# Griffan/FASTQuick

Measured on AMD Instinct MI355X. Metric: paired_150bp_reads_aligned_per_sec, higher is better.
Workload: dtype u32

## Files before the change

fastquick_amd/csrc/fq_align.cpp:

```cpp
#include <algorithm>
#include <atomic>
#include <ctime>
#include <chrono>
#include <climits>
#include <cstdint>
#include <cmath>
#include <cstdio>
#include <cstdlib>
#include <cstring>
#include <memory>
#include <string>
#include <unordered_map>
#include <mutex>
#include <thread>
#include <vector>
#include <pthread.h>
#include <sched.h>

#include "../../include/fastquick_amd.h"
#include "fq_backend.h"
#include "fq_index.h"
#include "fq_pipeline.h"
#include "fq_pool.h"
#include "fq_text_batch.h"
// ... 385 lines not shown
  else if (k == "device_turns") c->kn.device_turns = (int)v;
  else if (k == "device_turn_min") c->kn.device_turn_min = v;
  else if (k == "device_turn_slots") c->kn.device_turn_slots = (int)std::max<int64_t>(1, v);
  else if (k == "gap_round2_waves") c->kn.gap_round2_waves = (int)v;
  else if (k == "gap_round2_lane_major") c->kn.gap_round2_lane_major = (int)v;
  else if (k == "gap_round1_refill") c->kn.gap_round1_refill = (int)v;
  else if (k == "gap_round2_refill") c->kn.gap_round2_refill = (int)v;
  else if (k == "sw_wave_max") c->kn.sw_wave_max = (int)v;
  else if (k == "host_threads") c->kn.host_threads = (int)v;
  else if (k == "host_par_min") c->kn.host_par_min = (size_t)v;
  else if (k == "packed_bulk_min") c->kn.packed_bulk_min = v;
  else if (k == "md_mask_min") c->kn.md_mask_min = v;
  else if (k == "trace") c->kn.trace = (int)v;
  else if (k == "gap_order_asc") t->gap_order_asc = (int)v;
  else if (k == "gap_waves_per_cu") t->gap_waves_per_cu = (int)v;
  else if (k == "gap_coop_waves") t->gap_coop_waves = (int)v;
  else if (k == "gap_refill_min") t->gap_refill_min = (int)v;
  else if (k == "filter_no_turns") t->filter_no_turns = (int)v;
  else if (k == "prep_priority") t->prep_priority = (int)v;
  else if (k == "refine_lanes") t->refine_lanes = (int)v;
  else if (k == "gap_generic_opts") t->gap_generic_opts = (int)v;
  else if (k == "sw_serial_reverse") t->sw_serial_reverse = (int)v;
  else if (k == "width_both_strands") t->width_both_strands = (int)v;
  else if (k == "spin_sync") t->spin_sync = (int)v;
  else return FQ_EINVAL;
  return FQ_OK;
}

extern "C" void fq_stats_get(const fq_ctx_t *c, fq_stats_t *out) { if (c && out) *out = c->stats; }
extern "C" void fq_stats_reset(fq_ctx_t *c) { if (c) memset(&c->stats, 0, sizeof c->stats); }

#define CK(expr)                                                  \
  do {                                                            \
    if ((expr)) { c->err = std::string(#expr) + ": " + fqdev::last_error(); return FQ_ENODEV; } \
  } while (0)
#define CKM(expr)                                                 \
  do {                                                            \
    if (!(expr)) { c->err = std::string("out of device memory: ") + #expr; return FQ_ENOMEM; } \
  } while (0)

static int h2d_staged(fq_ctx *c, void *dst, const void *src, size_t bytes) {
  if (!bytes) return 0;
  void *p = c->arena.alloc(bytes);
  if (!p) { c->err = "out of pinned host memory"; return FQ_ENOMEM; }
  memcpy(p, src, bytes);
  if (fqdev::copy_pinned(dst, p, bytes, 1)) { c->err = std::string("h2d: ") + fqdev::last_error(); return FQ_ENODEV; }
// ... 712 lines not shown
    FqGapArgs gb = gap_args(c, b2, g, T2, (int32_t)cnt);
    gb.aln += (size_t)n2_total * T2.aln_cap; gb.n_aln += n2_total; gb.status += n2_total;
    gb.refill_min = 16;
    CK(fqdev::launch_gap(gb));
    CK(fqdev::stream_aux(0));
    n2_total += cnt;
  }
  CK(fqdev::stream_join());
  fqdev::time_end(FQ_K_GAP);
  *n2 = n2_total;
  return FQ_OK;
}

int stageA_search(Call &K) {
  fq_ctx *c = K.c;
  const fq_opts_t &o = c->o;
  SearchBufs &b = c->sb[0];
  const int n_search = K.n_search, max_len_all = K.max_len_all;
  c->st.aln.p = c->p_aln.p; c->st.aln.n = 0;
  par_assign(K.aln_off, (size_t)n_search + 1, (uint64_t)0, K.host_threads, K.par_min);
  par_assign(K.aln_n, (size_t)n_search, (uint32_t)0, K.host_threads, K.par_min);
  CKM(c->d_aoff.ensure((size_t)n_search + 1) && c->d_an.ensure((size_t)n_search + 1) && c->d_hits.ensure(1));
  CK(fqdev::dzero(c->d_an.p, ((size_t)n_search + 1) * 4));
  const SearchGeom g = {(max_len_all + 1 + 7) & ~7, (max_len_all + 1 + FQ_POS_PAD + 7) & ~7,
                        (c->maxdiff_lut[max_len_all] + 1) * o.s_mm + o.max_gapo * o.s_gapo + o.max_gape * o.s_gape + 1};
  const uint32_t exact_pool = (uint32_t)std::min<uint64_t>(4ull * (uint64_t)o.max_entries + 4096ull, 0x7fffffffull);
  const FqGapTier lane_tier = {c->kn.gap_pool, 32u, 0, 0, c->kn.gap_long_pops, c->kn.gap_long_always, 0, 0};
  const FqGapTier wave_tier = {262144u, 512u, 0, 1, 0u, 0, 0, 0}, exact_tier = {exact_pool, 8192u, 1, 1, 0u, 0, 0, 0};
  vector<FqGapTier> tiers;
  vector<size_t> chunk_reads;
  if (c->kn.gap_nogap_min >= 0 && !c->kn.gap_long_always && !(o.mode & FQ_MODE_NONSTOP) && c->kn.gap_pool <= 65535u) {
    FqGapTier t = lane_tier; t.nogap = 1; t.long_pops = 0; tiers.push_back(t); chunk_reads.push_back((size_t)8 << 20);
  }
  const size_t n_first_tiers = tiers.size();
  tiers.push_back(lane_tier); chunk_reads.push_back((size_t)8 << 20);
  tiers.push_back(wave_tier); chunk_reads.push_back((size_t)1 << 20);
  tiers.push_back(exact_tier); chunk_reads.push_back(4096);
  vector<int32_t> &work = c->cv.work, &next_work = c->cv.next_work;
  work.resize((size_t)n_search);
  parallel_chunks((size_t)n_search, K.host_threads, K.par_min, [&](size_t lo, size_t hi, int) { for (size_t s = lo; s < hi; ++s) work[s] = (int32_t)s; });
  bool ran_nogap = false;
  size_t n_hard = 0;
  vector<uint8_t> bound_of;
  for (size_t tier = 0; tier < tiers.size() && !work.empty(); ++tier) {
    FqGapTier T = tiers[tier];
    if (T.nogap && (int64_t)work.size() < c->kn.gap_nogap_min) continue;
    if (T.nogap) ran_nogap = true;
// ... 1367 lines not shown
```

fastquick_amd/csrc/fq_backend.h:

```cpp
#pragma once
#include "fq_kernels.h"
#include "fq_records.h"
#include "fq_frontend.h"
#include "fq_emit.h"
#include "fq_deflate.h"
#include "fq_sort.h"
#include "fq_bamin.h"

namespace fqdev {

struct State;
struct Tune {
  int gap_coop_waves = 0;
  int gap_waves_per_cu = 0, gap_refill_min = 0, gap_order_asc = 0, filter_no_turns = 0, refine_lanes = 0;
  int spin_sync = 0;
  int gap_generic_opts = 0;
  int width_both_strands = 0;
  int prep_priority = 0;
  int sw_serial_reverse = 0;
};
int runtime_configure(int hw_queues, int blocking_waits);
int device_count();
State *state_create(int device_ordinal);
void state_destroy(State *s);
int bind(State *s);
Tune *tune(State *s);
const char *last_error();
bool is_real_gpu();
void device_turn_begin(int slots = 1);
void device_turn_end();

void *dmalloc(size_t bytes);
void dfree(void *p);
void *hmalloc(size_t bytes);
void hfree(void *p);
int h2d(void *dst, const void *src, size_t bytes);
int d2h(void *dst, const void *src, size_t bytes);
int copy_pinned(void *dst, const void *src, size_t bytes, int to_device);
int d2d(void *dst, const void *src, size_t bytes);
int dzero(void *dst, size_t bytes);
int dfill(void *dst, int byte, size_t bytes);
int sync();
// ... 61 lines not shown
```

fastquick_amd/csrc/fq_device.hip:

```cpp
#include <hip/hip_runtime.h>
#include <hip/hip_ext.h>

#include <algorithm>
#include <condition_variable>
#include <atomic>
#include <cstdio>
#include <cstdlib>
#include <cstring>
#include <mutex>
#include <string>
#include <unordered_map>
#include <vector>
#include <sys/mman.h>
#include <sys/syscall.h>
#include <unistd.h>

#include "fq_backend.h"
#define FQ_PC_KERNELS
#include "fq_popcon.h"
#define FQ_SVD_KERNELS
#include "fq_svd.h"

namespace fqdev {

// ... 129 lines not shown
  }
  for (auto &p : s->pending) { (void)hipEventDestroy(p.a); (void)hipEventDestroy(p.b); }
  for (auto e : s->free_events) (void)hipEventDestroy(e);
  for (auto e : s->copy_done) if (e) (void)hipEventDestroy(e);
  if (s->prep_done) (void)hipEventDestroy(s->prep_done);
  if (s->scan_tmp) (void)hipFree(s->scan_tmp);
  if (s->cmp_cnt) (void)hipFree(s->cmp_cnt);
  if (s->cmp_off) (void)hipFree(s->cmp_off);
  if (s->stream) (void)hipStreamDestroy(s->stream);
  delete s;
}
Tune *tune(State *s) { return &s->tune; }
int bind(State *s) {
  if (!s) { g_err = "no device state"; return -3; }
  if (g_cur != s) { FQ_HIP(hipSetDevice(s->device)); g_cur = s; }
  return 0;
}

void *dmalloc(size_t bytes) {
  void *p = nullptr;
  if (hipMalloc(&p, bytes ? bytes : 16) != hipSuccess) { g_err = "hipMalloc failed (" + std::to_string(bytes) + " B)"; return nullptr; }
  return p;
}
void dfree(void *p) { if (p) (void)hipFree(p); }
static const size_t kRegisterMin = (size_t)4 << 20;
static std::mutex g_reg_mu;
static std::unordered_map<void *, size_t> g_registered;
static int device_numa_node(int dev) {
  static std::mutex mu;
  static std::unordered_map<int, int> cache;
  std::lock_guard<std::mutex> lk(mu);
  auto it = cache.find(dev);
  if (it != cache.end()) return it->second;
  int node = -1;
  char bus[64] = {0};
  if (hipDeviceGetPCIBusId(bus, (int)sizeof bus, dev) == hipSuccess) {
    for (char *c = bus; *c; ++c) if (*c >= 'A' && *c <= 'F') *c = (char)(*c - 'A' + 'a');
    const std::string path = std::string("/sys/bus/pci/devices/") + bus + "/numa_node";
    if (FILE *f = fopen(path.c_str(), "r")) { if (fscanf(f, "%d", &node) != 1) node = -1; fclose(f); }
  } else (void)hipGetLastError();
  cache[dev] = node;
  return node;
}
static void prefer_node(void *m, size_t len, int node) {
  if (node < 0 || node >= 1024) return;
  unsigned long mask[16] = {0};
  mask[node / (8 * sizeof(unsigned long))] |= 1ul << (node % (8 * sizeof(unsigned long)));
// ... 154 lines not shown
    g_cur->free_events.push_back(p.b);
  }
  g_cur->pending.swap(later);
}

static inline unsigned nblk(uint64_t n, unsigned b) { return (unsigned)((n + b - 1) / b); }

__global__ void __launch_bounds__(256) k_prep(FqPrepArgs a) {
  const int r = blockIdx.x * blockDim.x + threadIdx.x;
  if (r < a.n_reads) fq_prep_thread(a, r);
}
extern __shared__ __align__(16) unsigned char fq_dyn_lds[];
__global__ void __launch_bounds__(256) k_width(FqWidthArgs a) {
  uint8_t *seed_bits = (uint8_t *)fq_dyn_lds;
  const int w = blockIdx.x * blockDim.x + threadIdx.x;
  if (w < a.n_work) fq_width_read(a, w, seed_bits + threadIdx.x, 256);
}
__global__ void __launch_bounds__(256) k_width_strand(FqWidthArgs a) {
  uint8_t *seed_bits = (uint8_t *)fq_dyn_lds;
  const int xcd = blockIdx.x & 7, strand = xcd >> 2;
  const int q = (int)(blockIdx.x >> 3) * 4 + (xcd & 3);
  const int w = q * 256 + threadIdx.x;
  if (w < a.n_work) fq_width_strand(a, w, strand, seed_bits + threadIdx.x, 256);
}
struct FqQueueFetch {
  uint32_t *cursor;
  int n_work;
  __device__ uint32_t operator()(uint32_t n) const { return atomicAdd(cursor, n); }
};
#if defined(FQ_GAP_WPE)
#define FQ_GAP_OCC __attribute__((amdgpu_waves_per_eu(FQ_GAP_WPE, FQ_GAP_WPE)))
#else
#define FQ_GAP_OCC
#endif
#if defined(FQ_NOGAP_WPE)
#define FQ_NOGAP_OCC __attribute__((amdgpu_waves_per_eu(FQ_NOGAP_WPE, FQ_NOGAP_WPE)))
#define FQ_NOGAP_WAVES_PER_CU (4 * FQ_NOGAP_WPE)
#else
#define FQ_NOGAP_OCC FQ_GAP_OCC
#define FQ_NOGAP_WAVES_PER_CU 16
#endif
struct FqQueueFetch2 {
  uint32_t *cursor;
  const uint32_t *split;
  uint32_t n_work;
  int pref, seg, n_seg;
// ... 21 lines not shown
}
__global__ void __launch_bounds__(64) FQ_NOGAP_OCC k_gap_nogap_lds(FqGapArgs a) {
  uint16_t *heads = (uint16_t *)fq_dyn_lds;
  FqGapStoreLds st = {heads + threadIdx.x, 64, (uint32_t *)(heads + 64 * a.o.n_buckets) + threadIdx.x};
  fq_gap_lanes<true>(a, st, FQ_LANE_FETCH(a), (int)(blockIdx.x * 64 + threadIdx.x));
}
__global__ void __launch_bounds__(64) FQ_GAP_OCC k_gap_persist_stock(FqGapArgs a) {
  uint16_t *heads = (uint16_t *)fq_dyn_lds;
  FqGapStoreLds st = {heads + threadIdx.x, 64, (uint32_t *)(heads + 64 * a.o.n_buckets) + threadIdx.x};
  fq_gap_lanes<false, FqOptsStock>(a, st, FQ_LANE_FETCH(a), (int)(blockIdx.x * 64 + threadIdx.x));
}
__global__ void __launch_bounds__(64) FQ_NOGAP_OCC k_gap_nogap_stock(FqGapArgs a) {
  uint16_t *heads = (uint16_t *)fq_dyn_lds;
  FqGapStoreLds st = {heads + threadIdx.x, 64, (uint32_t *)(heads + 64 * a.o.n_buckets) + threadIdx.x};
  fq_gap_lanes<true, FqOptsStock>(a, st, FQ_LANE_FETCH(a), (int)(blockIdx.x * 64 + threadIdx.x));
}
__global__ void __launch_bounds__(64) k_gap_persist(FqGapArgs a) {
  FqGapStoreGlobal st = {nullptr, {}};
  fq_gap_lanes<false>(a, st, FQ_LANE_FETCH(a), (int)(blockIdx.x * 64 + threadIdx.x));
}
__global__ void __launch_bounds__(64) k_gap_coop(FqGapArgs a) {
  __shared__ uint32_t heads[2 * FQ_MAX_BUCKETS];
  fq_gap_coop_wave(a, heads, FqQueueFetch{a.queue, a.n_work}, (int)blockIdx.x);
}
__global__ void __launch_bounds__(256) k_sa(FqSaArgs a) {
  const uint64_t q = (uint64_t)blockIdx.x * blockDim.x + threadIdx.x;
  if (q < a.n_rows) fq_sa_thread(a, q);
}
template <bool PACKED>
__device__ __forceinline__ uint8_t fq_trace_get(const uint8_t *trace, int W, int j, int i) {
  if (!PACKED) return trace[(size_t)j * W + i];
  return (uint8_t)((trace[(size_t)j * ((W + 1) >> 1) + (i >> 1)] >> (4 * (i & 1))) & 15);
}
template <bool PACKED>
__device__ int fq_global_align_wave(const uint8_t *s1, int len1, const uint8_t *s2, int len2, int band, int gap_end,
                                    int *RM, int *RI, int *RD, uint8_t *trace, uint8_t *ops, int *n_ops, int *fi, int *fj) {
  const int lane = threadIdx.x;
  if (len1 == 0 || len2 == 0) { *n_ops = 0; return 0; }
  const FqBand g = fq_band(len1, len2, band, gap_end);
  if (lane == 0) {
    FqCell left;
    left.M = 0; left.I = left.D = FQ_NEG_INF;
    RM[0] = 0; RI[0] = RD[0] = FQ_NEG_INF;
    for (int i = 1; i < g.b1; ++i) {
      uint8_t tb;
      left = fq_band_row0(g, left, tb);
// ... 695 lines not shown
  if (t < a.n_rows) fq_trim_thread(a, t);
}
int launch_trim(const FqTrimArgs &a) {
  FQ_PRE();
  if (a.n_rows <= 0) return 0;
  hipLaunchKernelGGL(k_trim, dim3(nblk((uint64_t)a.n_rows, 256)), dim3(256), 0, g_stream, a);
  FQ_HIP(hipGetLastError());
  return 0;
}
__global__ void __launch_bounds__(256) k_trim_all(FqTrimAllArgs a) {
  const int r = blockIdx.x * blockDim.x + threadIdx.x;
  if (r < a.n_reads) fq_trim_all_thread(a, r);
}
int launch_trim_all(const FqTrimAllArgs &a) {
  FQ_PRE();
  if (a.n_reads <= 0) return 0;
  hipLaunchKernelGGL(k_trim_all, dim3(nblk((uint64_t)a.n_reads, 256)), dim3(256), 0, g_stream, a);
  FQ_HIP(hipGetLastError());
  return 0;
}
int launch_width(const FqWidthArgs &a) {
  FQ_PRE();
  if (a.n_work <= 0) return 0;
  hipEvent_t e0, e1;
  kernel_events(FQ_K_WIDTH_KERNEL, &e0, &e1);
  if (!g_cur->tune.width_both_strands) {
    const unsigned per_strand = nblk((uint64_t)a.n_work, 256);
    const unsigned grid = ((per_strand + 3) / 4) * 8;
    hipExtLaunchKernelGGL(k_width_strand, dim3(grid), dim3(256), (size_t)a.o.seed_len * 256, g_stream, e0, e1, 0, a);
  } else
  hipExtLaunchKernelGGL(k_width, dim3(nblk((uint64_t)a.n_work, 256)), dim3(256), (size_t)2 * (size_t)a.o.seed_len * 256, g_stream, e0, e1, 0, a);
  FQ_HIP(hipGetLastError());
  return 0;
}
__global__ void __launch_bounds__(256) k_order_count(const uint8_t *bid_end, int n, int n_hard, uint32_t *cnt) {
  __shared__ uint32_t h[FQ_ORDER_KEYS];
  if (threadIdx.x < FQ_ORDER_KEYS) h[threadIdx.x] = 0;
  __syncthreads();
  const int w = blockIdx.x * blockDim.x + threadIdx.x;
  if (w < n) atomicAdd(&h[fq_order_key(bid_end, w, n_hard)], 1u);
  __syncthreads();
  if (threadIdx.x < FQ_ORDER_KEYS && h[threadIdx.x]) atomicAdd(&cnt[threadIdx.x], h[threadIdx.x]);
}
__global__ void __launch_bounds__(256) k_order_scatter(const uint8_t *bid_end, int n, int n_hard, uint32_t *cnt, int32_t *order, int asc) {
  __shared__ uint32_t h[FQ_ORDER_KEYS], base[FQ_ORDER_KEYS];
  if (threadIdx.x < FQ_ORDER_KEYS) h[threadIdx.x] = 0;
  __syncthreads();
  const int w = blockIdx.x * blockDim.x + threadIdx.x;
  int key = 0;
  uint32_t rank = 0;
  if (w < n) { key = fq_order_key(bid_end, w, n_hard); rank = atomicAdd(&h[key], 1u); }
  __syncthreads();
// ... 72 lines not shown
  hipEvent_t e0, e1;
  kernel_events(a.tier.nogap ? FQ_K_GAP_NOGAP : FQ_K_GAP_KERNEL, &e0, &e1);
  if (a.tier.coop) {
    hipExtLaunchKernelGGL(k_gap_coop, dim3((unsigned)gap_lane_slots(a)), dim3(64), 0, g_stream, e0, e1, 0, a);
  } else {
    const size_t lds = (size_t)64 * (size_t)a.o.n_buckets * 2 + (size_t)64 * FQ_COLD_N * 4;
    const unsigned grid = (unsigned)gap_lane_slots(a) / 64u;
    if (a.tier.exact) { g_err = "launch_gap: the exact tier is the wavefront kernel's"; return -1; }
    const bool stock = FqOptsStock::matches(a.o) && !g_cur->tune.gap_generic_opts;
    if (a.tier.pool_cap <= 65535u && a.tier.nogap) hipExtLaunchKernelGGL(stock ? k_gap_nogap_stock : k_gap_nogap_lds, dim3(grid), dim3(64), lds, g_stream, e0, e1, 0, a);
    else if (a.tier.pool_cap <= 65535u) hipExtLaunchKernelGGL(stock ? k_gap_persist_stock : k_gap_persist_lds, dim3(grid), dim3(64), lds, g_stream, e0, e1, 0, a);
    else hipExtLaunchKernelGGL(k_gap_persist, dim3(grid), dim3(64), 0, g_stream, e0, e1, 0, a);
  }
  FQ_HIP(hipGetLastError());
  return 0;
}
int launch_pack_aln(const FqAln *aln, const uint32_t *n_aln, const uint64_t *off, uint32_t cap, uint32_t n_work, FqAln *packed) {
  FQ_PRE();
  if (!n_work) return 0;
  hipLaunchKernelGGL(k_pack_aln, dim3(nblk(n_work, 256)), dim3(256), 0, g_stream, aln, n_aln, off, cap, n_work, packed);
  FQ_HIP(hipGetLastError());
  return 0;
}
int launch_sa(const FqSaArgs &a) {
  FQ_PRE();
  if (!a.n_rows) return 0;
  hipEvent_t e0, e1;
  kernel_events(FQ_K_SA_KERNEL, &e0, &e1);
  hipExtLaunchKernelGGL(k_sa, dim3(nblk(a.n_rows, 256)), dim3(256), 0, g_stream, e0, e1, 0, a);
  FQ_HIP(hipGetLastError());
  return 0;
}
static const size_t kLdsBudget = 150 * 1024;
int launch_sw(const FqSwArgs &a) {
  FQ_PRE();
  if (a.n_task <= 0) return 0;
  const FqSwLds L(a.RL, a.QL);
  if (L.bytes(false) > kLdsBudget) { g_err = "SW window too large for LDS (" + std::to_string(a.RL) + " bases)"; return -5; }
  FqSwArgs b = a;
  b.trace_in_lds = (L.bytes(true) <= kLdsBudget && a.n_task <= 256) ? 1 : 0;
  b.serial_reverse = g_cur->tune.sw_serial_reverse;
  hipEvent_t e0, e1;
  kernel_events(FQ_K_SW_KERNEL, &e0, &e1);
  hipExtLaunchKernelGGL(k_sw_wave, dim3((unsigned)a.n_task), dim3(64), L.bytes(b.trace_in_lds), g_stream, e0, e1, 0, b);
  FQ_HIP(hipGetLastError());
  ++dp_launches[b.trace_in_lds ? FQ_DP_SW_WAVE_LDS : FQ_DP_SW_WAVE_GLOBAL];
  return 0;
}
__global__ void __launch_bounds__(64) k_sw_thread(FqSwArgs a) {
// ... 50 lines not shown
FQ_REC_KERNEL(k_pair_scatter, fq_pair_scatter_thread)
FQ_REC_KERNEL(k_xa_count, fq_xa_count_thread)
FQ_REC_KERNEL(k_xa_fill, fq_xa_fill_thread)
FQ_REC_KERNEL(k_sw_plan, fq_sw_plan_thread)
FQ_REC_KERNEL(k_sw_fill, fq_sw_fill_thread)
FQ_REC_KERNEL(k_rec_gather, fq_rec_gather_thread)
FQ_REC_KERNEL(k_rec_scatter, fq_rec_scatter_thread)
FQ_REC_KERNEL(k_ref_count, fq_ref_count_thread)
FQ_REC_KERNEL(k_ref_fill, fq_ref_fill_thread)
FQ_REC_KERNEL(k_ref_apply, fq_ref_apply_thread)
FQ_REC_KERNEL(k_md_rec, fq_md_rec_thread)
FQ_REC_KERNEL(k_md_mask, fq_md_mask_piece)
FQ_REC_KERNEL(k_flat_count, fq_flat_count_thread)
FQ_REC_KERNEL(k_flat_fill, fq_flat_fill_thread)
int launch_rec(int op, const FqRecArgs &a, int64_t n) {
  FQ_PRE();
  if (n <= 0) return 0;
  if (n > 0x7fffffff) { g_err = "record stage: more than 2^31 items"; return -5; }
  typedef void (*Kern)(FqRecArgs, int);
  static const Kern kerns[FQ_ROP_COUNT] = {k_rec_init, k_rec_nocc, k_enum_plan, k_enum_fill, k_main_hit, k_compact_idx, k_pair_rec, k_pair_gather, k_pair_scatter,
                                           k_xa_count, k_xa_fill, k_sw_plan, k_sw_fill, k_rec_gather, k_rec_scatter, k_ref_count, k_ref_fill, k_ref_apply,
                                           k_md_rec, k_md_mask, k_flat_count, k_flat_fill};
  if (op < 0 || op >= FQ_ROP_COUNT) { g_err = "record stage: unknown operation"; return -1; }
  hipEvent_t e0, e1;
  kernel_events(op == FQ_ROP_MD || op == FQ_ROP_MD_MASK ? FQ_K_MD_KERNEL : FQ_K_REC_KERNEL, &e0, &e1);
  hipExtLaunchKernelGGL(kerns[op], dim3(nblk((uint64_t)n, 256)), dim3(256), 0, g_stream, e0, e1, 0, a, (int)n);
  FQ_HIP(hipGetLastError());
  return 0;
}
__global__ void __launch_bounds__(256) k_sam_len(FqSamArgs a, int n) {
  const int i = blockIdx.x * blockDim.x + threadIdx.x;
  if (i < n) fq_sam_len_thread(a, i);
}
__global__ void __launch_bounds__(256) k_sam_fill(FqSamArgs a, int n) {
  const int i = blockIdx.x * blockDim.x + threadIdx.x;
  if (i < n) fq_sam_fill_thread(a, i);
}
__global__ void __launch_bounds__(256) k_sam_body(FqSamArgs a, int n, int pieces) {
  const uint64_t t = (uint64_t)blockIdx.x * blockDim.x + threadIdx.x;
  int idx, c;
  if (t < 0x100000000ull) { idx = (int)((uint32_t)t / (uint32_t)pieces); c = (int)((uint32_t)t - (uint32_t)idx * (uint32_t)pieces); }
  else { idx = (int)(t / (uint64_t)pieces); c = (int)(t % (uint64_t)pieces); }
  if (idx < n) fq_sam_body_piece(a, idx, c);
}
int launch_sam(int op, const FqSamArgs &a, int64_t n) {
  FQ_PRE();
  if (n <= 0) return 0;
  if (n > 0x7fffffff) { g_err = "SAM text: more than 2^31 records"; return -5; }
  hipEvent_t e0, e1;
// ... 620 lines not shown
```

fastquick_amd/csrc/fq_kernels.h:

```cpp
#pragma once
#include "fq_common.h"

#define FQ_LAMBDA_INLINE __attribute__((always_inline))
#if defined(__HIP_DEVICE_COMPILE__)
#define FQ_POPC64(x) __popcll(x)
#define FQ_POPC32(x) __popc(x)
#define FQ_CTZ32(x) (__ffs((int)(x)) - 1)
#define FQ_C_STRIPE_OFF ((size_t)(blockIdx.x & (FQ_C_STRIPES - 1)) * FQ_C_STRIDE)
#define FQ_ATOMIC_ADD64(p, v) atomicAdd((unsigned long long *)(p) + FQ_C_STRIPE_OFF, (unsigned long long)(v))
#define FQ_ATOMIC_MAX64(p, v) atomicMax((unsigned long long *)(p) + FQ_C_STRIPE_OFF, (unsigned long long)(v))
#define FQ_LOAD_RELAXED(p) __hip_atomic_load((p), __ATOMIC_RELAXED, __HIP_MEMORY_SCOPE_AGENT)
#define FQ_ATOMIC_MAX32(p, v) do { const int fq_v_ = (int)(v); if (fq_v_ > FQ_LOAD_RELAXED((const int *)(p))) atomicMax((int *)(p), fq_v_); } while (0)
#define FQ_WAVE_COUNT(p, pred)                                                                                      \
  do {                                                                                                              \
    const unsigned long long m_ = __ballot((pred) ? 1 : 0);                                                         \
    if ((pred) && __lane_id() == (unsigned)(__ffsll((long long)m_) - 1)) atomicAdd((unsigned long long *)(p) + FQ_C_STRIPE_OFF, (unsigned long long)__popcll(m_)); \
  } while (0)
#else
#define FQ_WAVE_COUNT(p, pred) do { if (pred) *(p) += 1; } while (0)
#define FQ_LOAD_RELAXED(p) (*(p))
#define FQ_ATOMIC_MAX32(p, v) (*(p) = *(p) > (int32_t)(v) ? *(p) : (int32_t)(v))
#define FQ_ATOMIC_MAX64(p, v) (*(p) = *(p) > (uint64_t)(v) ? *(p) : (uint64_t)(v))
#define FQ_POPC64(x) __builtin_popcountll(x)
#define FQ_POPC32(x) __builtin_popcount(x)
// ... 51 lines not shown
  const bool vl = l != 0xffffffffu && !(single_base && l == seq_len);
  const uint32_t ak = k >= primary ? k - 1 : k, al = l >= primary ? l - 1 : l;
  if (k == l) return vk ? 1u : 0u;
  if (vk && vl) return (ak >> 7) == (al >> 7) ? 1u : 2u;
  return (vk ? 1u : 0u) + (vl ? 1u : 0u);
}

FQ_HD uint32_t fq_sa_lookup(const FqFM &f, uint32_t k, uint32_t *steps) {
  uint32_t sa = 0;
  while (k % f.sa_intv != 0) {
    ++sa;
    if (k == f.primary) { k = 0; continue; }
    const uint32_t ka = fq_adj(f, k);
    const FqOccBlk *b = f.blk + (ka >> 6);
    const uint64_t hi = b->hi, lo = b->lo;
    const int sh = 63 - (int)(ka & 63);
    const int c = (int)((hi >> sh) & 1) << 1 | (int)((lo >> sh) & 1);
    const uint64_t m = ~0ull << sh;
    const uint64_t x = ((c & 2) ? hi : ~hi) & ((c & 1) ? lo : ~lo) & m;
    k = f.L2[c] + b->cnt[c] + (uint32_t)FQ_POPC64(x);
  }
  *steps += sa;
  return sa + f.sa[k / f.sa_intv];
}

FQ_HD uint32_t fq_pick2(uint32_t x1, uint32_t x0, int a) { const uint32_t m = 0u - (uint32_t)(a & 1); return (x1 & m) | (x0 & ~m); }
FQ_HD uint64_t fq_pick2p(uint64_t x1, uint64_t x0, int a) { const uint64_t m = 0ull - (uint64_t)(a & 1); return (x1 & m) | (x0 & ~m); }
FQ_HD uint32_t fq_sel4v(uint32_t v0, uint32_t v1, uint32_t v2, uint32_t v3, int c) {
  const uint32_t lo = (c & 1) ? v1 : v0, hi = (c & 1) ? v3 : v2;
  return (c & 2) ? hi : lo;
}
FQ_HD uint32_t fq_sel4(const uint32_t *v, int c) { return fq_sel4v(v[0], v[1], v[2], v[3], c & 3); }

struct FqBlkRaw { uint32_t c0, c1, c2, c3; uint32_t lo0, lo1, hi0, hi1; uint32_t mk0, mk1; bool valid; };
FQ_HD FqBlkRaw fq_blk_none() {
  FqBlkRaw r;
  r.valid = false;
  r.c0 = r.c1 = r.c2 = r.c3 = 0; r.lo0 = r.lo1 = r.hi0 = r.hi1 = 0; r.mk0 = r.mk1 = 0;
  return r;
}
FQ_HD FqBlkRaw fq_blk_load(const FqOccBlk *blk, uint32_t primary, uint32_t k) {
  FqBlkRaw r = fq_blk_none();
  r.valid = k != 0xffffffffu;
  if (r.valid) {
    k = k >= primary ? k - 1 : k;
    const FqOccBlk *b = blk + (k >> 6);
// ... 592 lines not shown
        if (c < 4) {
          touches += fq_touch2(f, k - 1, l, true);
          uint32_t ok, ol;
          fq_occ1_pair(f, k - 1, l, c, &ok, &ol);
          k = f.L2[c] + ok + 1;
          l = f.L2[c] + ol;
        }
        if (k > l || c > 3) { k = 0; l = f.seq_len; ++bid; }
        const uint32_t wcur = l - k + 1;
        const uint32_t seedbits = (use_seed && i >= seed_off) ? (uint32_t)seed_bits[(i - seed_off) * seed_bits_stride] << 6 : 0u;
        wv[j] = wcur;
        pv[j] = seedbits | (uint32_t)(bid < 31 ? bid : 31) | (i >= 1 && wcur == wprev ? 1u << 5 : 0u) | (uint32_t)c << 12;
        wprev = wcur;
      }
    }
    FqU4 q;
    q.x = wv[0]; q.y = wv[1]; q.z = wv[2]; q.w = wv[3];
    *(FqU4 *)(owa + i0) = q;
    q.x = wv[4]; q.y = wv[5]; q.z = wv[6]; q.w = wv[7];
    *(FqU4 *)(owa + i0 + 4) = q;
    q.x = pv[0] | pv[1] << 16; q.y = pv[2] | pv[3] << 16; q.z = pv[4] | pv[5] << 16; q.w = pv[6] | pv[7] << 16;
    *(FqU4 *)(pra + i0) = q;
  }
  A.bid_end[2 * w + a] = (uint8_t)(bid < 255 ? bid : 255);
  if (a == 0) {
    const uint32_t md = A.maxdiff_lut[v.len];
    FqGapWork gw;
    gw.r = r;
    gw.meta = (uint32_t)v.len | md << 16 | (namb > (int)md ? 1u << 24 : 0u);
    A.winfo[w] = gw;
  }
  FQ_ATOMIC_ADD64(&A.counters[FQ_C_OCC_WIDTH], touches);
}

#define FQ_ORDER_KEYS 32
FQ_HD int fq_order_key(const uint8_t *bid_end, int w, int n_hard) {
  const int a = bid_end[2 * w], b = bid_end[2 * w + 1];
  int k = a < b ? a : b;
  if (k > FQ_ORDER_KEYS / 4 - 1) k = FQ_ORDER_KEYS / 4 - 1;
  return (b <= a ? 0 : FQ_ORDER_KEYS / 2) + (w < n_hard ? FQ_ORDER_KEYS / 4 : 0) + k;
}

struct FqGapArgs {
  FqDevIndex ix;
  FqKOpts o;
  int32_t n_work;
// ... 987 lines not shown
template <class Fetch>
FQ_HD void fq_gap_coop_wave(const FqGapArgs &A, uint32_t *heads, Fetch fetch, int wave_slot) {
  FqGapCoop C(A, heads, wave_slot);
  uint32_t rounds = 0;
  for (;;) {
    uint32_t wq = 0;
    if (FQ_LANE_ID() == 0) wq = fetch(1u);
    wq = FQ_READLANE32(wq, 0);
    if (wq >= (uint32_t)A.n_work) break;
    rounds += C.run(A.order ? A.order[wq] : (int)wq);
  }
  if (FQ_LANE_ID() == 0) { FQ_ATOMIC_MAX64(&A.counters[FQ_C_MAXTRIPS], rounds); FQ_ATOMIC_ADD64(&A.counters[FQ_C_SUMTRIPS], rounds); }
}

struct FqSaArgs {
  FqDevIndex ix;
  const FqAln *aln;
  const uint32_t *aln_len;
  const uint64_t *row_off;
  uint32_t n_aln;
  uint64_t n_rows;
  uint32_t *pos;
  uint64_t *counters;
};
FQ_HD void fq_sa_thread(const FqSaArgs &A, uint64_t q) {
  uint32_t lo = 0, hi = A.n_aln;
  while (hi - lo > 1) {
    const uint32_t mid = (lo + hi) >> 1;
    if (A.row_off[mid] <= q) lo = mid; else hi = mid;
  }
  const FqAln h = A.aln[lo];
  const uint32_t row = h.k + (uint32_t)(q - A.row_off[lo]);
  const int a = (int)(h.info >> 24) & 1;
  uint32_t steps = 0, p;
  if (a) p = fq_sa_lookup(A.ix.fm[0], row, &steps);
  else p = A.ix.fm[1].seq_len - (fq_sa_lookup(A.ix.fm[1], row, &steps) + A.aln_len[lo]);
  A.pos[q] = p;
  FQ_ATOMIC_ADD64(&A.counters[FQ_C_OCC_SA], steps);
}
#define FQ_GAP_O 26
#define FQ_GAP_E 9
#define FQ_GAP_END 5
#define FQ_BAND 50
FQ_HD int fq_sm_maq(int a, int b) { return (a > 3 || b > 3) ? -13 : (a == b ? 11 : -19); }

struct FqCell { int M, I, D; };
FQ_HD int fq_pick_M(const FqCell &p, int sc, uint8_t &t) {
  if (p.M >= p.I) { if (p.M >= p.D) { t = FQ_OP_M; return p.M + sc; } t = FQ_OP_D; return p.D + sc; }
  if (p.I > p.D) { t = FQ_OP_I; return p.I + sc; }
  t = FQ_OP_D; return p.D + sc;
}
FQ_HD int fq_pick_gap(int m, int g, int ext, uint8_t &from_m) {
  if (m - FQ_GAP_O > g) { from_m = 1; return m - FQ_GAP_O - ext; }
  from_m = 0; return g - ext;
}

struct FqRowsArr {
  FqCell *c;
  FQ_HD FqCell get(int i) const { return c[i]; }
// ... 579 lines not shown
```

fastquick_amd/csrc/fq_records.h:

```cpp
#pragma once
#include "fq_kernels.h"
#include "../../include/fastquick_amd.h"

struct alignas(64) FqDRec {
  uint32_t pos, sa, c1, c2;
  int32_t score;
  int32_t sidx;
  int16_t len, full_len, clip_len, main_aln;
  uint8_t type, strand, filtered, extra_flag;
  uint8_t n_mm, n_gapo, n_gape, mapQ;
  uint8_t seQ, revived, has_md, pad0;
  uint16_t nm, n_cigar;
  uint32_t cig_off;
  uint32_t multi_off, n_multi;
  int32_t md_len;
};
static_assert(sizeof(FqDRec) == 64, "one record per cache line");

struct FqSwCand { int32_t sp, k; };
struct FqRefTgt { int32_t idx, multi; };
#define FQ_RNG_CHUNK_PAIRS 16
#define FQ_PAIR_LANE_ROWS 64u
#define FQ_CIG_CAP 64

// ... 3 lines not shown
  uint32_t max_occ, multi_cap;
  int32_t n_multi, N_multi, max_isize, s_mm, is_sw;
  const int32_t *pair_list;
  const FqSurvInfo *surv;
  const int32_t *len_trim;
  const int32_t *full_len;
  int32_t *sub_surv_max;
  const FqAln *hits;
  const uint64_t *aoff;
  const uint32_t *an;
  const uint8_t *maxdiff_lut;
  const int32_t *g_log_n;
  FqDRec *rec;
  uint32_t *nocc;
  uint16_t *ntop;
  uint8_t *enumerated;
  uint32_t *qfirst;
  uint64_t *row0;
  uint32_t *pq_cnt, *prow_cnt;
  const uint64_t *pq, *prow;
  FqAln *qaln; uint32_t *qlen; uint64_t *qoff;
  uint64_t n_q, n_rows;
  const uint32_t *pos;
  uint64_t *counters;
  const uint64_t *rng_start;
  uint32_t *isz;
  uint8_t *cls;
  uint32_t *flag32;
  const uint64_t *off64;
  int32_t *list;
  uint64_t *pscratch;
  const FqPairIsize *pisize;
  const int32_t *plut;
  FqPairRead *g_reads;
  uint64_t *g_row0;
  const FqPairOut *g_out;
  int32_t n_list;
  uint32_t *xcnt;
  const uint64_t *xoff;
  fq_multi_t *multi;
  const fq_isize_t *iis;
  FqSwTask *swslot;
  uint32_t *swcnt;
  const uint64_t *swoff;
  FqSwTask *swtask; FqSwCand *swcand;
  FqDRec *g_rec;
// ... 147 lines not shown
    }
    const int s = A.surv[idx].sidx;
    fq_main_draws(x, A.hits + A.aoff[s], A.an[s]);
  }
  FqDRec p[2];
  for (int e = 0; e < 2; ++e) {
    const int idx = 2 * sp + e;
    p[e] = A.rec[idx];
    if (p[e].filtered) continue;
    const int s = p[e].sidx;
    const FqAln *a = s >= 0 ? A.hits + A.aoff[s] : nullptr;
    const uint32_t na = s >= 0 ? A.an[s] : 0u;
    if (!fq_main_choose(x, a, na, p[e])) {
      p[e].type = FQ_TYPE_NO_MATCH; p[e].c1 = p[e].c2 = 0;
      FQ_ATOMIC_ADD64(&A.counters[FQ_C_ERR_DRAW0], 1);
    }
    if (fq_rec_mapped(p[e])) {
      if (A.enumerated[idx]) {
        uint64_t row = A.row0[idx];
        for (int k = 0; k < p[e].main_aln; ++k) row += (uint64_t)(a[k].l - a[k].k) + 1;
        p[e].pos = A.pos[row + (p[e].sa - a[p[e].main_aln].k)];
      } else {
        uint32_t steps = 0;
        p[e].pos = p[e].strand ? fq_sa_lookup(A.ix.fm[0], p[e].sa, &steps) : A.ix.fm[1].seq_len - (fq_sa_lookup(A.ix.fm[1], p[e].sa, &steps) + (uint32_t)p[e].len);
        FQ_ATOMIC_ADD64(&A.counters[FQ_C_OCC_SA], steps);
        FQ_ATOMIC_ADD64(&A.counters[FQ_C_SA_DIRECT], 1);
      }
      p[e].seQ = p[e].mapQ = (uint8_t)fq_approx_mapq(A, p[e]);
    }
    A.rec[idx] = p[e];
  }
  if (A.single_end) return;
  A.isz[sp] = fq_isize_sample(p[0], p[1]);
  const uint32_t o0 = A.nocc[2 * sp], o1 = A.nocc[2 * sp + 1];
  uint8_t cls = 0;
  if (fq_rec_mapped(p[0]) && fq_rec_mapped(p[1]) && o0 <= A.max_occ && o1 <= A.max_occ)
    cls = (A.enumerated[2 * sp] && A.enumerated[2 * sp + 1] && (uint64_t)o0 + o1 <= FQ_PAIR_LANE_ROWS) ? 1 : 2;
  A.cls[sp] = cls;
  A.flag32[sp] = cls == 2 ? 1u : 0u;
  FQ_WAVE_COUNT(&A.counters[FQ_C_PAIRS_DEV], cls == 1);
}

FQ_HD void fq_compact_thread(const FqRecArgs &A, int i) {
  if (A.flag32[i]) A.list[A.off64[i]] = i;
}

FQ_HD FqPairRead fq_pair_read_of(const FqDRec &p) {
// ... 348 lines not shown
```

Baseline: 765.1 million.

## Cache full suffix-array position table and batch width-kernel stores into whole lines

Adds a lazily built, per-index device table holding the suffix-array position and step count for every row, so SA lookups become one load instead of an LF-mapping walk. Separately adds a width kernel variant that buffers four 8-element groups in registers and writes them as whole 128-byte lines, and pads the search geometry strides to multiples of 32 so that variant is allowed. The table costs device memory and a one-time build with a host sync. The buffered stores raise register pressure.

After: 775.6 million (median of 4 runs). No clear change (+1.4%).

```diff
diff --git a/fastquick_amd/csrc/fq_align.cpp b/fastquick_amd/csrc/fq_align.cpp
--- a/fastquick_amd/csrc/fq_align.cpp
+++ b/fastquick_amd/csrc/fq_align.cpp
@@ -431,6 +431,8 @@
   else if (k == "gap_generic_opts") t->gap_generic_opts = (int)v;
   else if (k == "sw_serial_reverse") t->sw_serial_reverse = (int)v;
   else if (k == "width_both_strands") t->width_both_strands = (int)v;
+  else if (k == "width_store") t->width_store = (int)v;
+  else if (k == "sa_table") t->sa_table = (int)v;
   else if (k == "spin_sync") t->spin_sync = (int)v;
   else return FQ_EINVAL;
   return FQ_OK;
@@ -1189,7 +1191,7 @@
   par_assign(K.aln_n, (size_t)n_search, (uint32_t)0, K.host_threads, K.par_min);
   CKM(c->d_aoff.ensure((size_t)n_search + 1) && c->d_an.ensure((size_t)n_search + 1) && c->d_hits.ensure(1));
   CK(fqdev::dzero(c->d_an.p, ((size_t)n_search + 1) * 4));
-  const SearchGeom g = {(max_len_all + 1 + 7) & ~7, (max_len_all + 1 + FQ_POS_PAD + 7) & ~7,
+  const SearchGeom g = {(max_len_all + 1 + 31) & ~31, (max_len_all + 1 + FQ_POS_PAD + 31) & ~31,
                         (c->maxdiff_lut[max_len_all] + 1) * o.s_mm + o.max_gapo * o.s_gapo + o.max_gape * o.s_gape + 1};
   const uint32_t exact_pool = (uint32_t)std::min<uint64_t>(4ull * (uint64_t)o.max_entries + 4096ull, 0x7fffffffull);
   const FqGapTier lane_tier = {c->kn.gap_pool, 32u, 0, 0, c->kn.gap_long_pops, c->kn.gap_long_always, 0, 0};
diff --git a/fastquick_amd/csrc/fq_backend.h b/fastquick_amd/csrc/fq_backend.h
--- a/fastquick_amd/csrc/fq_backend.h
+++ b/fastquick_amd/csrc/fq_backend.h
@@ -18,6 +18,8 @@
   int width_both_strands = 0;
   int prep_priority = 0;
   int sw_serial_reverse = 0;
+  int width_store = 1;
+  int sa_table = 1;
 };
 int runtime_configure(int hw_queues, int blocking_waits);
 int device_count();
diff --git a/fastquick_amd/csrc/fq_device.hip b/fastquick_amd/csrc/fq_device.hip
--- a/fastquick_amd/csrc/fq_device.hip
+++ b/fastquick_amd/csrc/fq_device.hip
@@ -175,7 +175,8 @@
   if (hipMalloc(&p, bytes ? bytes : 16) != hipSuccess) { g_err = "hipMalloc failed (" + std::to_string(bytes) + " B)"; return nullptr; }
   return p;
 }
-void dfree(void *p) { if (p) (void)hipFree(p); }
+static void sa_table_drop(const void *blk);
+void dfree(void *p) { if (p) { sa_table_drop(p); (void)hipFree(p); } }
 static const size_t kRegisterMin = (size_t)4 << 20;
 static std::mutex g_reg_mu;
 static std::unordered_map<void *, size_t> g_registered;
@@ -376,6 +377,13 @@
   const int q = (int)(blockIdx.x >> 3) * 4 + (xcd & 3);
   const int w = q * 256 + threadIdx.x;
   if (w < a.n_work) fq_width_strand(a, w, strand, seed_bits + threadIdx.x, 256);
+}
+__global__ void __launch_bounds__(256) k_width_strand_seg(FqWidthArgs a) {
+  uint8_t *seed_bits = (uint8_t *)fq_dyn_lds;
+  const int xcd = blockIdx.x & 7, strand = xcd >> 2;
+  const int q = (int)(blockIdx.x >> 3) * 4 + (xcd & 3);
+  const int w = q * 256 + threadIdx.x;
+  if (w < a.n_work) fq_width_strand_seg(a, w, strand, seed_bits + threadIdx.x, 256);
 }
 struct FqQueueFetch {
   uint32_t *cursor;
@@ -443,6 +451,14 @@
 __global__ void __launch_bounds__(64) k_gap_coop(FqGapArgs a) {
   __shared__ uint32_t heads[2 * FQ_MAX_BUCKETS];
   fq_gap_coop_wave(a, heads, FqQueueFetch{a.queue, a.n_work}, (int)blockIdx.x);
+}
+__global__ void __launch_bounds__(256) k_sa_table(FqFM f, uint32_t *pos, uint16_t *steps, uint32_t *too_long) {
+  const uint64_t row = (uint64_t)blockIdx.x * blockDim.x + threadIdx.x;
+  if (row > (uint64_t)f.seq_len) return;
+  uint32_t st = 0;
+  pos[row] = fq_sa_lookup(f, (uint32_t)row, &st);
+  steps[row] = (uint16_t)st;
+  if (st > 0xffffu) atomicAdd(too_long, 1u);
 }
 __global__ void __launch_bounds__(256) k_sa(FqSaArgs a) {
   const uint64_t q = (uint64_t)blockIdx.x * blockDim.x + threadIdx.x;
@@ -1184,12 +1200,14 @@
 int launch_width(const FqWidthArgs &a) {
   FQ_PRE();
   if (a.n_work <= 0) return 0;
+  const bool seg = g_cur->tune.width_store != 0;
+  if (!g_cur->tune.width_both_strands && seg && (a.wstride % 32 != 0 || a.pstride % 32 != 0)) { g_err = "launch_width: whole-line stores need wstride % 32 == 0 and pstride % 32 == 0"; return -1; }
   hipEvent_t e0, e1;
   kernel_events(FQ_K_WIDTH_KERNEL, &e0, &e1);
   if (!g_cur->tune.width_both_strands) {
     const unsigned per_strand = nblk((uint64_t)a.n_work, 256);
     const unsigned grid = ((per_strand + 3) / 4) * 8;
-    hipExtLaunchKernelGGL(k_width_strand, dim3(grid), dim3(256), (size_t)a.o.seed_len * 256, g_stream, e0, e1, 0, a);
+    hipExtLaunchKernelGGL(seg ? k_width_strand_seg : k_width_strand, dim3(grid), dim3(256), (size_t)a.o.seed_len * 256, g_stream, e0, e1, 0, a);
   } else
   hipExtLaunchKernelGGL(k_width, dim3(nblk((uint64_t)a.n_work, 256)), dim3(256), (size_t)2 * (size_t)a.o.seed_len * 256, g_stream, e0, e1, 0, a);
   FQ_HIP(hipGetLastError());
@@ -1308,9 +1326,55 @@
   FQ_HIP(hipGetLastError());
   return 0;
 }
-int launch_sa(const FqSaArgs &a) {
-  FQ_PRE();
-  if (!a.n_rows) return 0;
+struct SaTable { uint32_t *pos[2] = {nullptr, nullptr}; uint16_t *steps[2] = {nullptr, nullptr}; bool ok = false; };
+static std::mutex g_sa_mu;
+static std::unordered_map<const void *, SaTable> g_sa_tables;
+static std::atomic<int> g_sa_n{0};
+static void sa_table_free(SaTable &t) {
+  for (int j = 0; j < 2; ++j) { if (t.pos[j]) (void)hipFree(t.pos[j]); if (t.steps[j]) (void)hipFree(t.steps[j]); t.pos[j] = nullptr; t.steps[j] = nullptr; }
+  t.ok = false;
+}
+static void sa_table_drop(const void *blk) {
+  if (g_sa_n.load(std::memory_order_relaxed) == 0) return;
+  std::lock_guard<std::mutex> lk(g_sa_mu);
+  auto it = g_sa_tables.find(blk);
+  if (it == g_sa_tables.end()) return;
+  sa_table_free(it->second);
+  g_sa_tables.erase(it);
+  --g_sa_n;
+}
+static FqSaTab sa_table_for(const FqDevIndex &ix) {
+  FqSaTab out = {{nullptr, nullptr}, {nullptr, nullptr}};
+  if (!g_cur->tune.sa_table || !ix.fm[0].blk || !ix.fm[1].blk) return out;
+  std::lock_guard<std::mutex> lk(g_sa_mu);
+  auto it = g_sa_tables.find(ix.fm[0].blk);
+  if (it == g_sa_tables.end()) {
+    SaTable t;
+    uint32_t *too_long = nullptr;
+    bool ok = hipMalloc((void **)&too_long, 4) == hipSuccess && hipMemsetAsync(too_long, 0, 4, g_stream) == hipSuccess;
+    for (int j = 0; j < 2 && ok; ++j) {
+      const size_t rows = (size_t)ix.fm[j].seq_len + 1;
+      ok = hipMalloc((void **)&t.pos[j], rows * 4) == hipSuccess && hipMalloc((void **)&t.steps[j], rows * 2) == hipSuccess;
+      if (!ok) break;
+      hipLaunchKernelGGL(k_sa_table, dim3(nblk(rows, 256)), dim3(256), 0, g_stream, ix.fm[j], t.pos[j], t.steps[j], too_long);
+      ok = hipGetLastError() == hipSuccess;
+    }
+    uint32_t n_long = 0;
+    ok = ok && hipMemcpyAsync(&n_long, too_long, 4, hipMemcpyDeviceToHost, g_stream) == hipSuccess && hipStreamSynchronize(g_stream) == hipSuccess && n_long == 0;
+    if (!ok) { (void)hipGetLastError(); (void)hipStreamSynchronize(g_stream); sa_table_free(t); }
+    if (too_long) (void)hipFree(too_long);
+    t.ok = ok;
+    it = g_sa_tables.emplace(ix.fm[0].blk, t).first;
+    ++g_sa_n;
+  }
+  if (it->second.ok) for (int j = 0; j < 2; ++j) { out.pos[j] = it->second.pos[j]; out.steps[j] = it->second.steps[j]; }
+  return out;
+}
+int launch_sa(const FqSaArgs &a_in) {
+  FQ_PRE();
+  if (!a_in.n_rows) return 0;
+  FqSaArgs a = a_in;
+  a.tab = sa_table_for(a.ix);
   hipEvent_t e0, e1;
   kernel_events(FQ_K_SA_KERNEL, &e0, &e1);
   hipExtLaunchKernelGGL(k_sa, dim3(nblk(a.n_rows, 256)), dim3(256), 0, g_stream, e0, e1, 0, a);
@@ -1407,9 +1471,11 @@
                                            k_xa_count, k_xa_fill, k_sw_plan, k_sw_fill, k_rec_gather, k_rec_scatter, k_ref_count, k_ref_fill, k_ref_apply,
                                            k_md_rec, k_md_mask, k_flat_count, k_flat_fill};
   if (op < 0 || op >= FQ_ROP_COUNT) { g_err = "record stage: unknown operation"; return -1; }
+  FqRecArgs b = a;
+  if (op == FQ_ROP_MAIN_HIT) b.sa_tab = sa_table_for(a.ix);
   hipEvent_t e0, e1;
   kernel_events(op == FQ_ROP_MD || op == FQ_ROP_MD_MASK ? FQ_K_MD_KERNEL : FQ_K_REC_KERNEL, &e0, &e1);
-  hipExtLaunchKernelGGL(kerns[op], dim3(nblk((uint64_t)n, 256)), dim3(256), 0, g_stream, e0, e1, 0, a, (int)n);
+  hipExtLaunchKernelGGL(kerns[op], dim3(nblk((uint64_t)n, 256)), dim3(256), 0, g_stream, e0, e1, 0, b, (int)n);
   FQ_HIP(hipGetLastError());
   return 0;
 }
diff --git a/fastquick_amd/csrc/fq_kernels.h b/fastquick_amd/csrc/fq_kernels.h
--- a/fastquick_amd/csrc/fq_kernels.h
+++ b/fastquick_amd/csrc/fq_kernels.h
@@ -97,6 +97,11 @@
   }
   *steps += sa;
   return sa + f.sa[k / f.sa_intv];
+}
+struct FqSaTab { const uint32_t *pos[2]; const uint16_t *steps[2]; };
+FQ_HD uint32_t fq_sa_pos(const FqDevIndex &ix, const FqSaTab &t, int which, uint32_t k, uint32_t *steps) {
+  if (t.pos[which] && k <= ix.fm[which].seq_len) { *steps += t.steps[which][k]; return t.pos[which][k]; }
+  return fq_sa_lookup(ix.fm[which], k, steps);
 }
 
 FQ_HD uint32_t fq_pick2(uint32_t x1, uint32_t x0, int a) { const uint32_t m = 0u - (uint32_t)(a & 1); return (x1 & m) | (x0 & ~m); }
@@ -735,6 +740,122 @@
     q.x = pv[0] | pv[1] << 16; q.y = pv[2] | pv[3] << 16; q.z = pv[4] | pv[5] << 16; q.w = pv[6] | pv[7] << 16;
     *(FqU4 *)(pra + i0) = q;
   }
+  A.bid_end[2 * w + a] = (uint8_t)(bid < 255 ? bid : 255);
+  if (a == 0) {
+    const uint32_t md = A.maxdiff_lut[v.len];
+    FqGapWork gw;
+    gw.r = r;
+    gw.meta = (uint32_t)v.len | md << 16 | (namb > (int)md ? 1u << 24 : 0u);
+    A.winfo[w] = gw;
+  }
+  FQ_ATOMIC_ADD64(&A.counters[FQ_C_OCC_WIDTH], touches);
+}
+
+FQ_HD void fq_store16(void *p, uint32_t x, uint32_t y, uint32_t z, uint32_t w) {
+  FqU4 q;
+  q.x = x; q.y = y; q.z = z; q.w = w;
+  *(FqU4 *)p = q;
+}
+FQ_HD void fq_width_strand_seg(const FqWidthArgs &A, int w, int a, uint8_t *seed_bits, int seed_bits_stride) {
+  const int s = A.work ? A.work[w] : w;
+  const int r = A.read_list[s];
+  FqReadView v = {A.seq + (size_t)r * (size_t)A.stride, A.len_trim[r]};
+  uint32_t *owa = A.wfull + (size_t)w * 2 * (size_t)A.wstride + (size_t)a * (size_t)A.wstride;
+  FqPos *pra = A.prec + (size_t)w * 2 * (size_t)A.pstride + (size_t)a * (size_t)A.pstride;
+  const FqFM &f = A.ix.fm[a];
+  uint32_t touches = 0;
+  const bool use_seed = v.len > A.o.seed_len;
+  const int seed_off = v.len - A.o.seed_len;
+  uint32_t k = 0, l = f.seq_len, wprev = 0;
+  int bid = 0;
+  if (use_seed) {
+    uint64_t seed8 = 0;
+    for (int i = 0; i < A.o.seed_len; ++i) {
+      if ((i & 7) == 0 && i + 8 <= A.o.seed_len) memcpy(&seed8, v.row + (A.o.seed_len - 8 - i), 8);
+      const bool fast = (i | 7) < A.o.seed_len;
+      int c;
+      if (fast) { const int c0 = (int)fq_nt4_fast((uint32_t)(seed8 >> (8 * (7 - (i & 7)))) & 0xffu); c = (a && c0 < 4) ? 3 - c0 : c0; }
+      else c = fq_base(v, a, seed_off + i);
+      if (c < 4) {
+        touches += fq_touch2(f, k - 1, l, true);
+        uint32_t ok, ol;
+        fq_occ1_pair(f, k - 1, l, c, &ok, &ol);
+        k = f.L2[c] + ok + 1;
+        l = f.L2[c] + ol;
+      }
+      if (k > l || c > 3) { k = 0; l = f.seq_len; ++bid; }
+      const uint32_t wcur = l - k + 1;
+      seed_bits[i * seed_bits_stride] = (uint8_t)((uint32_t)(bid < 31 ? bid : 31) | (i >= 1 && wcur == wprev ? 1u << 5 : 0u));
+      wprev = wcur;
+    }
+  }
+  k = 0; l = f.seq_len; wprev = 0; bid = 0;
+  int namb = 0;
+  uint32_t wst[24], pst[12];
+#pragma unroll
+  for (int j = 0; j < 24; ++j) wst[j] = 0;
+#pragma unroll
+  for (int j = 0; j < 12; ++j) pst[j] = 0;
+  for (int i0 = 0; i0 < v.len; i0 += 8) {
+    uint32_t wv[8], pv[8];
+    uint64_t bases8 = 0;
+    const bool whole = i0 + 8 <= v.len;
+    if (whole) memcpy(&bases8, v.row + (v.len - 8 - i0), 8);
+#pragma unroll
+    for (int j = 0; j < 8; ++j) {
+      const int i = i0 + j;
+      wv[j] = 0; pv[j] = 0;
+      if (i < v.len) {
+        int c;
+        if (whole) { const int c0 = (int)fq_nt4_fast((uint32_t)(bases8 >> (8 * (7 - j))) & 0xffu); c = (a && c0 < 4) ? 3 - c0 : c0; }
+        else c = fq_base(v, a, i);
+        namb += c > 3;
+        if (c < 4) {
+          touches += fq_touch2(f, k - 1, l, true);
+          uint32_t ok, ol;
+          fq_occ1_pair(f, k - 1, l, c, &ok, &ol);
+          k = f.L2[c] + ok + 1;
+          l = f.L2[c] + ol;
+        }
+        if (k > l || c > 3) { k = 0; l = f.seq_len; ++bid; }
+        const uint32_t wcur = l - k + 1;
+        const uint32_t seedbits = (use_seed && i >= seed_off) ? (uint32_t)seed_bits[(i - seed_off) * seed_bits_stride] << 6 : 0u;
+        wv[j] = wcur;
+        pv[j] = seedbits | (uint32_t)(bid < 31 ? bid : 31) | (i >= 1 && wcur == wprev ? 1u << 5 : 0u) | (uint32_t)c << 12;
+        wprev = wcur;
+      }
+    }
+    const uint32_t q0 = pv[0] | pv[1] << 16, q1 = pv[2] | pv[3] << 16, q2 = pv[4] | pv[5] << 16, q3 = pv[6] | pv[7] << 16;
+    const int g = (i0 >> 3) & 3;
+    if (g < 3) {
+#pragma unroll
+      for (int t = 0; t < 3; ++t)
+        if (g == t) {
+#pragma unroll
+          for (int j = 0; j < 8; ++j) wst[t * 8 + j] = wv[j];
+          pst[t * 4] = q0; pst[t * 4 + 1] = q1; pst[t * 4 + 2] = q2; pst[t * 4 + 3] = q3;
+        }
+    } else {
+#pragma unroll
+      for (int t = 0; t < 3; ++t) {
+        fq_store16(owa + i0 - (3 - t) * 8, wst[t * 8], wst[t * 8 + 1], wst[t * 8 + 2], wst[t * 8 + 3]);
+        fq_store16(owa + i0 - (3 - t) * 8 + 4, wst[t * 8 + 4], wst[t * 8 + 5], wst[t * 8 + 6], wst[t * 8 + 7]);
+      }
+      fq_store16(owa + i0, wv[0], wv[1], wv[2], wv[3]);
+      fq_store16(owa + i0 + 4, wv[4], wv[5], wv[6], wv[7]);
+#pragma unroll
+      for (int t = 0; t < 3; ++t) fq_store16(pra + i0 - (3 - t) * 8, pst[t * 4], pst[t * 4 + 1], pst[t * 4 + 2], pst[t * 4 + 3]);
+      fq_store16(pra + i0, q0, q1, q2, q3);
+    }
+  }
+  const int ng = (v.len + 7) >> 3, left = ng & 3, base = (ng & ~3) * 8;
+#pragma unroll
+  for (int t = 0; t < 3; ++t)
+    if (t < left) {
+      fq_store16(owa + base + t * 8, wst[t * 8], wst[t * 8 + 1], wst[t * 8 + 2], wst[t * 8 + 3]);
+      fq_store16(owa + base + t * 8 + 4, wst[t * 8 + 4], wst[t * 8 + 5], wst[t * 8 + 6], wst[t * 8 + 7]);
+      fq_store16(pra + base + t * 8, pst[t * 4], pst[t * 4 + 1], pst[t * 4 + 2], pst[t * 4 + 3]);
+    }
   A.bid_end[2 * w + a] = (uint8_t)(bid < 255 ? bid : 255);
   if (a == 0) {
     const uint32_t md = A.maxdiff_lut[v.len];
@@ -1768,6 +1889,7 @@
   uint64_t n_rows;
   uint32_t *pos;
   uint64_t *counters;
+  FqSaTab tab;
 };
 FQ_HD void fq_sa_thread(const FqSaArgs &A, uint64_t q) {
   uint32_t lo = 0, hi = A.n_aln;
@@ -1779,8 +1901,8 @@
   const uint32_t row = h.k + (uint32_t)(q - A.row_off[lo]);
   const int a = (int)(h.info >> 24) & 1;
   uint32_t steps = 0, p;
-  if (a) p = fq_sa_lookup(A.ix.fm[0], row, &steps);
-  else p = A.ix.fm[1].seq_len - (fq_sa_lookup(A.ix.fm[1], row, &steps) + A.aln_len[lo]);
+  if (a) p = fq_sa_pos(A.ix, A.tab, 0, row, &steps);
+  else p = A.ix.fm[1].seq_len - (fq_sa_pos(A.ix, A.tab, 1, row, &steps) + A.aln_len[lo]);
   A.pos[q] = p;
   FQ_ATOMIC_ADD64(&A.counters[FQ_C_OCC_SA], steps);
 }
diff --git a/fastquick_amd/csrc/fq_records.h b/fastquick_amd/csrc/fq_records.h
--- a/fastquick_amd/csrc/fq_records.h
+++ b/fastquick_amd/csrc/fq_records.h
@@ -49,6 +49,7 @@
   FqAln *qaln; uint32_t *qlen; uint64_t *qoff;
   uint64_t n_q, n_rows;
   const uint32_t *pos;
+  FqSaTab sa_tab;
   uint64_t *counters;
   const uint64_t *rng_start;
   uint32_t *isz;
@@ -242,7 +243,7 @@
         p[e].pos = A.pos[row + (p[e].sa - a[p[e].main_aln].k)];
       } else {
         uint32_t steps = 0;
-        p[e].pos = p[e].strand ? fq_sa_lookup(A.ix.fm[0], p[e].sa, &steps) : A.ix.fm[1].seq_len - (fq_sa_lookup(A.ix.fm[1], p[e].sa, &steps) + (uint32_t)p[e].len);
+        p[e].pos = p[e].strand ? fq_sa_pos(A.ix, A.sa_tab, 0, p[e].sa, &steps) : A.ix.fm[1].seq_len - (fq_sa_pos(A.ix, A.sa_tab, 1, p[e].sa, &steps) + (uint32_t)p[e].len);
         FQ_ATOMIC_ADD64(&A.counters[FQ_C_OCC_SA], steps);
         FQ_ATOMIC_ADD64(&A.counters[FQ_C_SA_DIRECT], 1);
       }
```
